# IST-DASLab/gptq-gguf-toolkit

Hardware: AMD Instinct MI355X
Metric: Mparams/s GPTQ-quantized (higher is better)
Workload: dtype f32; 1 GPU; llama3-8b-block-q4k: 7 Linears of one block (218.1 M params), 128x2048-token calibration fed per sequence through the package's BlockSchedule, block_size 128, rel_damp 0.01, nstep 20; calib_seqs_per_rank=128, parallelism=calib-dp1+matrix-fanout, owners=rank0

## Files before the change

gptq-gguf-toolkit_amd/csrc/gq_gptq.hip:

```cpp
#include <atomic>
#include <mutex>
#include "gq_common.hpp"
#include "gq_gemm32.hpp"
#include "gq_walk.hpp"
#include <stdlib.h>

namespace gq {

constexpr int SEG = 128;
constexpr int SB = 16;
constexpr int SEG_WAVES = 8;
constexpr int SEG_LDS_BYTES = (SEG * 64 + SEG * SEG + 2 * SB * 64) * 4 + SEG * 8;

__device__ __forceinline__ float div_rcp64(float n, double rd) { return (float)((double)n * rd); }

struct BandTable {
    int32_t n;
    int32_t end64[GQ_BANDS_MAX];
    uint32_t info[GQ_BANDS_MAX];
    int64_t sm_off[GQ_BANDS_MAX];
};
template <bool BANDS> struct BandArg {};
template <> struct BandArg<true> { BandTable t; };

template <bool PERM, bool UNI = false, bool BANDS = false>
__global__ __launch_bounds__(SEG_WAVES * 64) void gptq_segment_kernel(
    float* W, int64_t C, const float* src, int64_t ld_src,
    const float* __restrict__ U, int64_t a, int len, int64_t R,
    const uint16_t* __restrict__ d, const uint8_t* __restrict__ s, const uint16_t* __restrict__ dmin,
    const uint8_t* __restrict__ m, int G, int is_signed, float qmin, float qmax,
    uint8_t* __restrict__ qweight, float* __restrict__ Err, int64_t ld_err, int64_t err_col0,
    const int32_t* __restrict__ perm, const float* __restrict__ uscale = nullptr,
    const float* __restrict__ uzero = nullptr,
    const float* __restrict__ Unext = nullptr,
    int npair = 1,
    BandArg<BANDS> bands = {}) {
    extern __shared__ __attribute__((aligned(16))) float seg_smem[];
    float* wl = seg_smem;
    float* Us = seg_smem + SEG * 64;
    float* ne = Us + SEG * SEG;
    double* rdiag = reinterpret_cast<double*>(ne + 2 * SB * 64);
    const int tid = threadIdx.x, lane = tid & 63, wid = tid >> 6;
    const int64_t row = (int64_t)blockIdx.x * 64 + lane;
    const bool live = row < R;
    const int64_t r = live ? row : 0;
    int64_t band_row0 = 0;
    if constexpr (BANDS) {
        static_assert(!PERM && !UNI, "bands are K-quants in natural column order");
        const BandTable& bt = bands.t;
        int k = 0;
        while (k + 1 < bt.n && (int)blockIdx.x >= bt.end64[k]) ++k;
        const uint32_t info = bt.info[k];
        G = (int)(info & 0xffu);
        is_signed = (int)((info >> 8) & 1u);
        qmin = (float)(int8_t)((info >> 16) & 0xffu);
        qmax = (float)(info >> 24);
        band_row0 = k ? (int64_t)bt.end64[k - 1] * 64 : 0;
        s += bt.sm_off[k];
        m += bt.sm_off[k];
    }
    for (int half = 0; half < npair; ++half) {
    if (half) {
        __syncthreads();
        a += SEG;
        src += SEG;
        err_col0 += SEG;
        Unext = nullptr;
    }
    auto load_u_rows = [&](int i_lo, int i_hi, int t0, int nthr) {
        for (int idx = t0; idx < (i_hi - i_lo) * (SEG / 4); idx += nthr) {
            const int i = i_lo + idx / (SEG / 4), j4 = (idx % (SEG / 4)) * 4;
            float4 v = make_float4(0.f, 0.f, 0.f, 0.f);
            if (j4 < len) v = *reinterpret_cast<const float4*>(U + (a + i) * C + a + j4);
            *reinterpret_cast<float4*>(Us + i * SEG + j4) = v;
        }
    };
    auto load_w_cols = [&](int j_lo, int j_hi, int w0, int nw) {
        const float* sp = src + r * ld_src;
        for (int j = j_lo + w0 * 4; j < j_hi; j += 4 * nw) {
            float4 v = *reinterpret_cast<const float4*>(sp + j);
            wl[(j + 0) * 64 + lane] = v.x;
            wl[(j + 1) * 64 + lane] = v.y;
            wl[(j + 2) * 64 + lane] = v.z;
            wl[(j + 3) * 64 + lane] = v.w;
        }
    };
    const int first = len < SB ? len : SB;
    if (tid < first) rdiag[tid] = 1.0 / (double)U[(a + tid) * C + a + tid];
    load_u_rows(0, first, tid, SEG_WAVES * 64);
    load_w_cols(0, first, wid, SEG_WAVES);
    const int64_t nsg = C / 256, ng = C / G;
    constexpr int NT = SEG / SB;
    float dst[PERM ? 1 : NT], dmt[PERM ? 1 : NT];
    double rdt[PERM ? 1 : NT];
    if constexpr (!PERM) {
        if (wid == 0) {
#pragma unroll
            for (int t = 0; t < NT; ++t) {
                const int64_t col0 = a + t * SB < a + len ? a + t * SB : a;
                if constexpr (UNI) {
                    dst[t] = uscale[r * ng + col0 / G];
                    dmt[t] = uzero[r * ng + col0 / G];
                } else if constexpr (BANDS) {
                    const int64_t rb = r - band_row0;
                    dst[t] = h2f(d[r * nsg + col0 / 256]) * ival(s[rb * ng + col0 / G], is_signed);
                    dmt[t] = h2f(dmin[r * nsg + col0 / 256]) * ival(m[rb * ng + col0 / G], is_signed);
                } else {
                    dst[t] = h2f(d[r * nsg + col0 / 256]) * ival(s[r * ng + col0 / G], is_signed);
                    dmt[t] = h2f(dmin[r * nsg + col0 / 256]) * ival(m[r * ng + col0 / G], is_signed);
                }
                rdt[t] = 1.0 / (double)(dst[t] < 1e-9f ? 1e-9f : dst[t]);
            }
        }
    }
    __syncthreads();
    if (wid != 0) {
        const int ht = tid - 64;
        if (ht >= first && ht < len) rdiag[ht] = 1.0 / (double)U[(a + ht) * C + a + ht];
        load_u_rows(first, len, ht, (SEG_WAVES - 1) * 64);
        load_w_cols(first, len, wid - 1, SEG_WAVES - 1);
    }

    const int ntile = len / SB;
#pragma unroll
    for (int t = 0; t < NT; ++t) {
        if (t >= ntile) break;
        const int i0 = t * SB;
        float* net = ne + (t & 1) * (SB * 64);
        if (wid == 0) {
            const int64_t col0 = a + i0;
            float ds = 0.f, dm = 0.f, dsv[PERM ? SB : 1], dmv[PERM ? SB : 1];
            double rden = 0.0, rdenv[PERM ? SB : 1];
            if constexpr (PERM) {
#pragma unroll
                for (int k = 0; k < SB; ++k) {
                    const int64_t pc = perm[col0 + k];
                    dsv[k] = h2f(d[r * nsg + pc / 256]) * ival(s[r * ng + pc / G], is_signed);
                    dmv[k] = h2f(dmin[r * nsg + pc / 256]) * ival(m[r * ng + pc / G], is_signed);
                    rdenv[k] = 1.0 / (double)(dsv[k] < 1e-9f ? 1e-9f : dsv[k]);
                }
            } else {
                ds = dst[t];
                dm = dmt[t];
                rden = rdt[t];
            }
            float wr[SB], nerr[SB], wq[SB];
            uint32_t qpack[4] = {0, 0, 0, 0};
#pragma unroll
            for (int k = 0; k < SB; ++k) wr[k] = wl[(i0 + k) * 64 + lane];
#pragma unroll
            for (int k = 0; k < SB; ++k) {
                const float* urow = Us + (i0 + k) * SEG + i0;
                if constexpr (PERM) { ds = dsv[k]; dm = dmv[k]; rden = rdenv[k]; }
                float q;
                if constexpr (UNI) {
                    q = clampf(rintf(div_rcp64(wr[k], rden) + dm), qmin, qmax);
                    wq[k] = ds * (q - dm);
                } else {
                    q = clampf(rintf(div_rcp64(wr[k] + dm, rden)), qmin, qmax);
                    wq[k] = dequantize1(q, ds, dm);
                }
                const float err = div_rcp64(wr[k] - wq[k], rdiag[i0 + k]);
                const uint8_t qb = is_signed ? (uint8_t)(int8_t)q : (uint8_t)q;
                qpack[k >> 2] |= (uint32_t)qb << (8 * (k & 3));
                const float nk = -err;
                nerr[k] = nk;
#pragma unroll
                for (int kk = k; kk < SB; ++kk) wr[kk] = wr[kk] + nk * urow[kk];
            }
#pragma unroll
            for (int k = 0; k < SB; ++k) net[k * 64 + lane] = nerr[k];
            if (live) {
                *reinterpret_cast<uint4*>(qweight + row * C + col0) =
                    make_uint4(qpack[0], qpack[1], qpack[2], qpack[3]);
                float* wp = W + row * C + col0;
                float* ep = Err + row * ld_err + err_col0 + i0;
#pragma unroll
                for (int k = 0; k < SB; k += 4) {
                    *reinterpret_cast<float4*>(wp + k) = make_float4(wq[k], wq[k + 1], wq[k + 2], wq[k + 3]);
                    *reinterpret_cast<float4*>(ep + k) =
                        make_float4(-nerr[k], -nerr[k + 1], -nerr[k + 2], -nerr[k + 3]);
                }
            }
        }
        if (wid != 0 && t > 0) {
            const float* nep = ne + ((t - 1) & 1) * (SB * 64);
            if (Unext != nullptr && wid == SEG_WAVES - 1) {
#pragma unroll
                for (int k = 0; k < SB; ++k) wl[(i0 - SB + k) * 64 + lane] = nep[k * 64 + lane];
            }
            int turn = 0;
            for (int j0 = i0 + SB; j0 < len; j0 += SB, ++turn) {
                if ((turn % (SEG_WAVES - 1)) + 1 != wid) continue;
                float wt[SB], nk[SB];
#pragma unroll
                for (int jj = 0; jj < SB; ++jj) wt[jj] = wl[(j0 + jj) * 64 + lane];
#pragma unroll
                for (int k = 0; k < SB; ++k) nk[k] = nep[k * 64 + lane];
#pragma unroll
                for (int k = 0; k < SB; ++k) {
                    const float* urow = Us + (i0 - SB + k) * SEG + j0;
#pragma unroll
                    for (int jj = 0; jj < SB; ++jj) wt[jj] = wt[jj] + nk[k] * urow[jj];
                }
#pragma unroll
                for (int jj = 0; jj < SB; ++jj) wl[(j0 + jj) * 64 + lane] = wt[jj];
            }
        }
        __syncthreads();
        if (i0 + SB < len) {
            constexpr int CPW = SB / SEG_WAVES;
            const int j0 = i0 + SB + wid * CPW;
            float wt[CPW];
#pragma unroll
            for (int jj = 0; jj < CPW; ++jj) wt[jj] = wl[(j0 + jj) * 64 + lane];
#pragma unroll
            for (int k = 0; k < SB; ++k) {
                const float nk = net[k * 64 + lane];
#pragma unroll
                for (int jj = 0; jj < CPW; ++jj) wt[jj] = wt[jj] + nk * Us[(i0 + k) * SEG + j0 + jj];
            }
#pragma unroll
            for (int jj = 0; jj < CPW; ++jj) wl[(j0 + jj) * 64 + lane] = wt[jj];
        }
        __syncthreads();
    }
    if (Unext != nullptr) {
        for (int idx = tid; idx < SEG * (SEG / 4); idx += SEG_WAVES * 64) {
            const int i = idx / (SEG / 4), j4 = (idx % (SEG / 4)) * 4;
            *reinterpret_cast<float4*>(Us + i * SEG + j4) = *reinterpret_cast<const float4*>(Unext + (int64_t)i * C + j4);
        }
        __syncthreads();
        const int rb = (wid & 1) * 32, cb = (wid >> 1) * 32;
        const int li = lane & 31, lk = lane >> 5;
        const float* nel = ne + ((ntile - 1) & 1) * (SB * 64);
        f32x16 acc;
#pragma unroll
        for (int e = 0; e < 16; ++e) acc[e] = 0.0f;
#pragma unroll 8
        for (int k0 = 0; k0 < SEG; k0 += 2) {
            const int k = k0 + lk;
            const float ev = (k < SEG - SB) ? wl[k * 64 + rb + li] : nel[(k - (SEG - SB)) * 64 + rb + li];
            acc = __builtin_amdgcn_mfma_f32_32x32x2f32(ev, Us[k * SEG + cb + li], acc, 0, 0, 0);
        }
        const int64_t r0 = (int64_t)blockIdx.x * 64 + rb + 4 * lk;
        float* wp = W + r0 * C + a + SEG + cb + li;
        float wv[16];
#pragma unroll
        for (int e = 0; e < 16; ++e) {
            const int ro = (e & 3) + 8 * (e >> 2);
            wv[e] = (r0 + ro < R) ? wp[(int64_t)ro * C] : 0.0f;
        }
#pragma unroll
        for (int e = 0; e < 16; ++e) {
            const int ro = (e & 3) + 8 * (e >> 2);
            if (r0 + ro < R) wp[(int64_t)ro * C] = wv[e] + acc[e];
        }
    }
    }
}

__global__ __launch_bounds__(256) void uniform_params_kernel(const float* __restrict__ x, int64_t R, int64_t ld, int G,
                                                             float maxq, int sym, float* __restrict__ scale,
                                                             float* __restrict__ zero, int64_t ng) {
    const int lane = threadIdx.x & 63;
    const int64_t row = (int64_t)blockIdx.x * 4 + (threadIdx.x >> 6);
    if (row >= R) return;
    const float* xr = x + row * ld;
    float mn = xr[0], mx = mn;
    for (int j = lane * 4; j < G; j += 256) {
        const float4 v = *reinterpret_cast<const float4*>(xr + j);
        mn = fminf(fminf(mn, v.x), fminf(v.y, fminf(v.z, v.w)));
        mx = fmaxf(fmaxf(mx, v.x), fmaxf(v.y, fmaxf(v.z, v.w)));
    }
#pragma unroll
    for (int o = 32; o > 0; o >>= 1) {
        mn = fminf(mn, __shfl_xor(mn, o));
        mx = fmaxf(mx, __shfl_xor(mx, o));
    }
    if (lane) return;
    if (sym) {
        mx = fmaxf(fabsf(mn), mx);
        if (mn < 0.0f) mn = -mx;
    }
    if (mn == mx) {
        mn = -1.0f;
        mx = 1.0f;
    }
    const float sc = (mx - mn) / maxq;
    scale[row * ng] = sc;
    zero[row * ng] = sym ? (maxq + 1.0f) / 2.0f : rintf(-mn / sc);
}

__global__ __launch_bounds__(256) void block_far_update_kernel(float* __restrict__ Wblk, int64_t ld_blk,
                                                               int64_t ncols, int64_t R,
                                                               const float* __restrict__ Err, int64_t ld_err,
                                                               int64_t e0, int n_i, const float* __restrict__ U,
                                                               int64_t C, int64_t a, int64_t cj0) {
    const int64_t total = R * ncols;
    for (int64_t t = (int64_t)blockIdx.x * blockDim.x + threadIdx.x; t < total;
         t += (int64_t)gridDim.x * blockDim.x) {
        const int64_t r = t / ncols, j = t % ncols;
        float w = Wblk[r * ld_blk + j];
        const float* e = Err + r * ld_err + e0;
        for (int i = 0; i < n_i; ++i) w = w + (-e[i]) * U[(a + i) * C + cj0 + j];
        Wblk[r * ld_blk + j] = w;
    }
}

__global__ __launch_bounds__(256) void copy2d_kernel(float* __restrict__ dst, int64_t ld_dst,
                                                     const float* __restrict__ src, int64_t ld_src, int64_t R,
                                                     int64_t ncols) {
    const int64_t total = R * ncols;
    for (int64_t t = (int64_t)blockIdx.x * blockDim.x + threadIdx.x; t < total;
         t += (int64_t)gridDim.x * blockDim.x) {
        const int64_t r = t / ncols, j = t % ncols;
        dst[r * ld_dst + j] = src[r * ld_src + j];
    }
}

int launch_trailing_update(float* Cmat, int64_t ldc, const float* A, int64_t lda, const float* B, int64_t ldb,
                           int64_t M, int64_t N, int64_t K, hipStream_t st) {
    ProfScope ps(PT_TRAILING, st);
    return launch_gemm32<false, 0, false>(Cmat, ldc, A, lda, B, ldb, M, N, K, st);
}

constexpr int LA = 8;
constexpr int LA_B = 128;

static std::atomic<int> g_far_enabled{1};
int far_helper_enable(int on) { return g_far_enabled.exchange(on ? 1 : 0); }

WalkOptions walk_options() {
    return WalkOptions{opt(OPT_la), opt(OPT_no_lookahead), opt(OPT_far_sync), opt(OPT_far_async_max_rows),
                       opt(OPT_far_async_min_sb), opt(OPT_far_wgs), opt(OPT_near64_maxn), g_far_enabled.load() != 0};
}

WalkPlan walk_plan(int64_t R, int64_t C, int block_size, WalkKind kind, int uniform_group, const WalkOptions& o) {
    WalkPlan p{};
    const int64_t B = p.B = block_size <= 0 || block_size > C ? C : block_size;
    p.la = (o.la >= 2 && o.la <= LA && o.la % 2 == 0) ? (int)o.la : LA;
    const int ug = kind == WalkKind::Uniform && uniform_group > 0 ? uniform_group : 0;
    p.lookahead = B == LA_B && !o.no_lookahead && (!ug || (p.la * B) % ug == 0);
    p.pair_look = p.lookahead && p.la % 2 == 0 && (!ug || 256 % ug == 0);
    p.ldE = p.lookahead ? (int64_t)LA * B : B;
    p.helper_ok = p.lookahead && o.helper_enabled && !o.far_sync && R % 128 == 0 && C % 128 == 0 &&
                  R <= o.far_async_max_rows && C >= o.far_async_min_sb * (int64_t)p.la * B;
    p.far_wgs = (int)o.far_wgs;
    p.near64_maxn = o.near64_maxn;
    const size_t blk = (size_t)R * (size_t)B * sizeof(float);
    const size_t err = blk * (B == LA_B ? 2 * (size_t)LA : 1);
    p.needs_blk = B > SEG || (B > 0 && 256 % B != 0);
    p.err_off[0] = 0;
    p.err_off[1] = B == LA_B ? blk * LA : 0;
    p.blk_off = err;
    p.panel_off = (err + (p.needs_blk ? blk : 0) + 255) & ~(size_t)255;
    p.total = err + (p.needs_blk ? blk : 0) + 256 + 256;
    return p;
}

size_t gptq_workspace_bytes(int64_t R, int64_t C, int block_size) {
    return walk_plan(R, C, block_size, WalkKind::KQuant, 0, walk_options()).total;
}
int gptq_uses_helper_stream(int64_t R, int64_t C, int block_size) {
    return walk_plan(R, C, block_size, WalkKind::KQuant, 0, walk_options()).helper_ok;
}

struct BandPlan {
    BandTable tbl;
    int q_type[GQ_BANDS_MAX];
    int64_t row_end[GQ_BANDS_MAX];
};

enum class ScaleSearch {
    None,
    UpFront,
    Lazy,
};

struct Walk {
    const WalkCall& c;
    WalkPlan p;
    TypeInfo ti;
    ScaleSearch search;
    float *err[2], *Wblk;
    unsigned* panel;
    int64_t ng, nsg;
    int gps;
    bool helper;
};
struct Block {
    int64_t c1, c2;
    int64_t sb, pos;
    int64_t S0, S1;
    bool single;
    float* Err;
};

static int walk_open(const WalkCall& c, Walk& w) {
    const bool uni = c.kind == WalkKind::Uniform;
    w.ti = TypeInfo{};
    if (uni) {
        w.ti.group = c.uni.group > 0 ? c.uni.group : (int)c.C;
        w.ti.qmax = (1 << c.uni.bits) - 1;
    } else if (c.kind == WalkKind::Bands) {
        w.ti.group = 16;
        for (int k = 0; k < c.bands->tbl.n; ++k) {
            TypeInfo tk;
            type_info(c.bands->q_type[k], tk);
            w.ti.k_search |= tk.k_search;
        }
    } else if (!type_info(c.q_type, w.ti)) GQ_FAIL(GQ_E_BAD_TYPE, "gq_gptq_quantize: unknown q_type %d", c.q_type);
    if (c.R <= 0 || c.C <= 0 || c.C % 256)
// ... 389 lines not shown
```

Baseline: 2432 Mparams/s.

## Hand over paired segment in LDS instead of reloading, add stamp profiling

Moves the segment kernel into its own header and changes the paired-block path (non-uniform quants). After the first 128-column block, the trailing update results for the partner block are written straight into the LDS working buffer, and the next U tile and its diagonal reciprocals are prefetched. The second half therefore skips its prologue reload and the extra barrier. The commit also adds an optional s_memtime stamp template parameter and a micro-profiler program. This removes global-memory round trips and a sync at the hand-over, at the cost of more complex LDS bookkeeping and higher register pressure.

```diff
diff --git a/gptq-gguf-toolkit_amd/csrc/gq_gptq.hip b/gptq-gguf-toolkit_amd/csrc/gq_gptq.hip
--- a/gptq-gguf-toolkit_amd/csrc/gq_gptq.hip
+++ b/gptq-gguf-toolkit_amd/csrc/gq_gptq.hip
@@ -3,262 +3,10 @@
 #include "gq_common.hpp"
 #include "gq_gemm32.hpp"
 #include "gq_walk.hpp"
+#include "gq_segment.hpp"
 #include <stdlib.h>
 
 namespace gq {
-
-constexpr int SEG = 128;
-constexpr int SB = 16;
-constexpr int SEG_WAVES = 8;
-constexpr int SEG_LDS_BYTES = (SEG * 64 + SEG * SEG + 2 * SB * 64) * 4 + SEG * 8;
-
-__device__ __forceinline__ float div_rcp64(float n, double rd) { return (float)((double)n * rd); }
-
-struct BandTable {
-    int32_t n;
-    int32_t end64[GQ_BANDS_MAX];
-    uint32_t info[GQ_BANDS_MAX];
-    int64_t sm_off[GQ_BANDS_MAX];
-};
-template <bool BANDS> struct BandArg {};
-template <> struct BandArg<true> { BandTable t; };
-
-template <bool PERM, bool UNI = false, bool BANDS = false>
-__global__ __launch_bounds__(SEG_WAVES * 64) void gptq_segment_kernel(
-    float* W, int64_t C, const float* src, int64_t ld_src,
-    const float* __restrict__ U, int64_t a, int len, int64_t R,
-    const uint16_t* __restrict__ d, const uint8_t* __restrict__ s, const uint16_t* __restrict__ dmin,
-    const uint8_t* __restrict__ m, int G, int is_signed, float qmin, float qmax,
-    uint8_t* __restrict__ qweight, float* __restrict__ Err, int64_t ld_err, int64_t err_col0,
-    const int32_t* __restrict__ perm, const float* __restrict__ uscale = nullptr,
-    const float* __restrict__ uzero = nullptr,
-    const float* __restrict__ Unext = nullptr,
-    int npair = 1,
-    BandArg<BANDS> bands = {}) {
-    extern __shared__ __attribute__((aligned(16))) float seg_smem[];
-    float* wl = seg_smem;
-    float* Us = seg_smem + SEG * 64;
-    float* ne = Us + SEG * SEG;
-    double* rdiag = reinterpret_cast<double*>(ne + 2 * SB * 64);
-    const int tid = threadIdx.x, lane = tid & 63, wid = tid >> 6;
-    const int64_t row = (int64_t)blockIdx.x * 64 + lane;
-    const bool live = row < R;
-    const int64_t r = live ? row : 0;
-    int64_t band_row0 = 0;
-    if constexpr (BANDS) {
-        static_assert(!PERM && !UNI, "bands are K-quants in natural column order");
-        const BandTable& bt = bands.t;
-        int k = 0;
-        while (k + 1 < bt.n && (int)blockIdx.x >= bt.end64[k]) ++k;
-        const uint32_t info = bt.info[k];
-        G = (int)(info & 0xffu);
-        is_signed = (int)((info >> 8) & 1u);
-        qmin = (float)(int8_t)((info >> 16) & 0xffu);
-        qmax = (float)(info >> 24);
-        band_row0 = k ? (int64_t)bt.end64[k - 1] * 64 : 0;
-        s += bt.sm_off[k];
-        m += bt.sm_off[k];
-    }
-    for (int half = 0; half < npair; ++half) {
-    if (half) {
-        __syncthreads();
-        a += SEG;
-        src += SEG;
-        err_col0 += SEG;
-        Unext = nullptr;
-    }
-    auto load_u_rows = [&](int i_lo, int i_hi, int t0, int nthr) {
-        for (int idx = t0; idx < (i_hi - i_lo) * (SEG / 4); idx += nthr) {
-            const int i = i_lo + idx / (SEG / 4), j4 = (idx % (SEG / 4)) * 4;
-            float4 v = make_float4(0.f, 0.f, 0.f, 0.f);
-            if (j4 < len) v = *reinterpret_cast<const float4*>(U + (a + i) * C + a + j4);
-            *reinterpret_cast<float4*>(Us + i * SEG + j4) = v;
-        }
-    };
-    auto load_w_cols = [&](int j_lo, int j_hi, int w0, int nw) {
-        const float* sp = src + r * ld_src;
-        for (int j = j_lo + w0 * 4; j < j_hi; j += 4 * nw) {
-            float4 v = *reinterpret_cast<const float4*>(sp + j);
-            wl[(j + 0) * 64 + lane] = v.x;
-            wl[(j + 1) * 64 + lane] = v.y;
-            wl[(j + 2) * 64 + lane] = v.z;
-            wl[(j + 3) * 64 + lane] = v.w;
-        }
-    };
-    const int first = len < SB ? len : SB;
-    if (tid < first) rdiag[tid] = 1.0 / (double)U[(a + tid) * C + a + tid];
-    load_u_rows(0, first, tid, SEG_WAVES * 64);
-    load_w_cols(0, first, wid, SEG_WAVES);
-    const int64_t nsg = C / 256, ng = C / G;
-    constexpr int NT = SEG / SB;
-    float dst[PERM ? 1 : NT], dmt[PERM ? 1 : NT];
-    double rdt[PERM ? 1 : NT];
-    if constexpr (!PERM) {
-        if (wid == 0) {
-#pragma unroll
-            for (int t = 0; t < NT; ++t) {
-                const int64_t col0 = a + t * SB < a + len ? a + t * SB : a;
-                if constexpr (UNI) {
-                    dst[t] = uscale[r * ng + col0 / G];
-                    dmt[t] = uzero[r * ng + col0 / G];
-                } else if constexpr (BANDS) {
-                    const int64_t rb = r - band_row0;
-                    dst[t] = h2f(d[r * nsg + col0 / 256]) * ival(s[rb * ng + col0 / G], is_signed);
-                    dmt[t] = h2f(dmin[r * nsg + col0 / 256]) * ival(m[rb * ng + col0 / G], is_signed);
-                } else {
-                    dst[t] = h2f(d[r * nsg + col0 / 256]) * ival(s[r * ng + col0 / G], is_signed);
-                    dmt[t] = h2f(dmin[r * nsg + col0 / 256]) * ival(m[r * ng + col0 / G], is_signed);
-                }
-                rdt[t] = 1.0 / (double)(dst[t] < 1e-9f ? 1e-9f : dst[t]);
-            }
-        }
-    }
-    __syncthreads();
-    if (wid != 0) {
-        const int ht = tid - 64;
-        if (ht >= first && ht < len) rdiag[ht] = 1.0 / (double)U[(a + ht) * C + a + ht];
-        load_u_rows(first, len, ht, (SEG_WAVES - 1) * 64);
-        load_w_cols(first, len, wid - 1, SEG_WAVES - 1);
-    }
-
-    const int ntile = len / SB;
-#pragma unroll
-    for (int t = 0; t < NT; ++t) {
-        if (t >= ntile) break;
-        const int i0 = t * SB;
-        float* net = ne + (t & 1) * (SB * 64);
-        if (wid == 0) {
-            const int64_t col0 = a + i0;
-            float ds = 0.f, dm = 0.f, dsv[PERM ? SB : 1], dmv[PERM ? SB : 1];
-            double rden = 0.0, rdenv[PERM ? SB : 1];
-            if constexpr (PERM) {
-#pragma unroll
-                for (int k = 0; k < SB; ++k) {
-                    const int64_t pc = perm[col0 + k];
-                    dsv[k] = h2f(d[r * nsg + pc / 256]) * ival(s[r * ng + pc / G], is_signed);
-                    dmv[k] = h2f(dmin[r * nsg + pc / 256]) * ival(m[r * ng + pc / G], is_signed);
-                    rdenv[k] = 1.0 / (double)(dsv[k] < 1e-9f ? 1e-9f : dsv[k]);
-                }
-            } else {
-                ds = dst[t];
-                dm = dmt[t];
-                rden = rdt[t];
-            }
-            float wr[SB], nerr[SB], wq[SB];
-            uint32_t qpack[4] = {0, 0, 0, 0};
-#pragma unroll
-            for (int k = 0; k < SB; ++k) wr[k] = wl[(i0 + k) * 64 + lane];
-#pragma unroll
-            for (int k = 0; k < SB; ++k) {
-                const float* urow = Us + (i0 + k) * SEG + i0;
-                if constexpr (PERM) { ds = dsv[k]; dm = dmv[k]; rden = rdenv[k]; }
-                float q;
-                if constexpr (UNI) {
-                    q = clampf(rintf(div_rcp64(wr[k], rden) + dm), qmin, qmax);
-                    wq[k] = ds * (q - dm);
-                } else {
-                    q = clampf(rintf(div_rcp64(wr[k] + dm, rden)), qmin, qmax);
-                    wq[k] = dequantize1(q, ds, dm);
-                }
-                const float err = div_rcp64(wr[k] - wq[k], rdiag[i0 + k]);
-                const uint8_t qb = is_signed ? (uint8_t)(int8_t)q : (uint8_t)q;
-                qpack[k >> 2] |= (uint32_t)qb << (8 * (k & 3));
-                const float nk = -err;
-                nerr[k] = nk;
-#pragma unroll
-                for (int kk = k; kk < SB; ++kk) wr[kk] = wr[kk] + nk * urow[kk];
-            }
-#pragma unroll
-            for (int k = 0; k < SB; ++k) net[k * 64 + lane] = nerr[k];
-            if (live) {
-                *reinterpret_cast<uint4*>(qweight + row * C + col0) =
-                    make_uint4(qpack[0], qpack[1], qpack[2], qpack[3]);
-                float* wp = W + row * C + col0;
-                float* ep = Err + row * ld_err + err_col0 + i0;
-#pragma unroll
-                for (int k = 0; k < SB; k += 4) {
-                    *reinterpret_cast<float4*>(wp + k) = make_float4(wq[k], wq[k + 1], wq[k + 2], wq[k + 3]);
-                    *reinterpret_cast<float4*>(ep + k) =
-                        make_float4(-nerr[k], -nerr[k + 1], -nerr[k + 2], -nerr[k + 3]);
-                }
-            }
-        }
-        if (wid != 0 && t > 0) {
-            const float* nep = ne + ((t - 1) & 1) * (SB * 64);
-            if (Unext != nullptr && wid == SEG_WAVES - 1) {
-#pragma unroll
-                for (int k = 0; k < SB; ++k) wl[(i0 - SB + k) * 64 + lane] = nep[k * 64 + lane];
-            }
-            int turn = 0;
-            for (int j0 = i0 + SB; j0 < len; j0 += SB, ++turn) {
-                if ((turn % (SEG_WAVES - 1)) + 1 != wid) continue;
-                float wt[SB], nk[SB];
-#pragma unroll
-                for (int jj = 0; jj < SB; ++jj) wt[jj] = wl[(j0 + jj) * 64 + lane];
-#pragma unroll
-                for (int k = 0; k < SB; ++k) nk[k] = nep[k * 64 + lane];
-#pragma unroll
-                for (int k = 0; k < SB; ++k) {
-                    const float* urow = Us + (i0 - SB + k) * SEG + j0;
-#pragma unroll
-                    for (int jj = 0; jj < SB; ++jj) wt[jj] = wt[jj] + nk[k] * urow[jj];
-                }
-#pragma unroll
-                for (int jj = 0; jj < SB; ++jj) wl[(j0 + jj) * 64 + lane] = wt[jj];
-            }
-        }
-        __syncthreads();
-        if (i0 + SB < len) {
-            constexpr int CPW = SB / SEG_WAVES;
-            const int j0 = i0 + SB + wid * CPW;
-            float wt[CPW];
-#pragma unroll
-            for (int jj = 0; jj < CPW; ++jj) wt[jj] = wl[(j0 + jj) * 64 + lane];
-#pragma unroll
-            for (int k = 0; k < SB; ++k) {
-                const float nk = net[k * 64 + lane];
-#pragma unroll
-                for (int jj = 0; jj < CPW; ++jj) wt[jj] = wt[jj] + nk * Us[(i0 + k) * SEG + j0 + jj];
-            }
-#pragma unroll
-            for (int jj = 0; jj < CPW; ++jj) wl[(j0 + jj) * 64 + lane] = wt[jj];
-        }
-        __syncthreads();
-    }
-    if (Unext != nullptr) {
-        for (int idx = tid; idx < SEG * (SEG / 4); idx += SEG_WAVES * 64) {
-            const int i = idx / (SEG / 4), j4 = (idx % (SEG / 4)) * 4;
-            *reinterpret_cast<float4*>(Us + i * SEG + j4) = *reinterpret_cast<const float4*>(Unext + (int64_t)i * C + j4);
-        }
-        __syncthreads();
-        const int rb = (wid & 1) * 32, cb = (wid >> 1) * 32;
-        const int li = lane & 31, lk = lane >> 5;
-        const float* nel = ne + ((ntile - 1) & 1) * (SB * 64);
-        f32x16 acc;
-#pragma unroll
-        for (int e = 0; e < 16; ++e) acc[e] = 0.0f;
-#pragma unroll 8
-        for (int k0 = 0; k0 < SEG; k0 += 2) {
-            const int k = k0 + lk;
-            const float ev = (k < SEG - SB) ? wl[k * 64 + rb + li] : nel[(k - (SEG - SB)) * 64 + rb + li];
-            acc = __builtin_amdgcn_mfma_f32_32x32x2f32(ev, Us[k * SEG + cb + li], acc, 0, 0, 0);
-        }
-        const int64_t r0 = (int64_t)blockIdx.x * 64 + rb + 4 * lk;
-        float* wp = W + r0 * C + a + SEG + cb + li;
-        float wv[16];
-#pragma unroll
-        for (int e = 0; e < 16; ++e) {
-            const int ro = (e & 3) + 8 * (e >> 2);
-            wv[e] = (r0 + ro < R) ? wp[(int64_t)ro * C] : 0.0f;
-        }
-#pragma unroll
-        for (int e = 0; e < 16; ++e) {
-            const int ro = (e & 3) + 8 * (e >> 2);
-            if (r0 + ro < R) wp[(int64_t)ro * C] = wv[e] + acc[e];
-        }
-    }
-    }
-}
 
 __global__ __launch_bounds__(256) void uniform_params_kernel(const float* __restrict__ x, int64_t R, int64_t ld, int G,
                                                              float maxq, int sym, float* __restrict__ scale,
diff --git a/gptq-gguf-toolkit_amd/csrc/gq_segment.hpp b/gptq-gguf-toolkit_amd/csrc/gq_segment.hpp
--- /dev/null
+++ b/gptq-gguf-toolkit_amd/csrc/gq_segment.hpp
@@ -0,0 +1,352 @@
+#pragma once
+#include "gq_common.hpp"
+#include "gq_gemm32.hpp"
+#include "../../include/gptq_gguf_levels.h"
+
+namespace gq {
+
+constexpr int SEG = 128;
+constexpr int SB = 16;
+constexpr int SEG_WAVES = 8;
+constexpr int SEG_LDS_BYTES = (SEG * 64 + SEG * SEG + 2 * SB * 64) * 4 + SEG * 8;
+
+__device__ __forceinline__ float div_rcp64(float n, double rd) { return (float)((double)n * rd); }
+
+struct BandTable {
+    int32_t n;
+    int32_t end64[GQ_BANDS_MAX];
+    uint32_t info[GQ_BANDS_MAX];
+    int64_t sm_off[GQ_BANDS_MAX];
+};
+template <bool BANDS> struct BandArg {};
+template <> struct BandArg<true> { BandTable t; };
+
+constexpr int SEG_STAMP_HALF = 24, SEG_NSTAMP = 2 * SEG_STAMP_HALF + 4;
+template <bool STAMP> struct StampArg {};
+template <> struct StampArg<true> { unsigned long long* buf; int wg; };
+
+template <bool PERM, bool UNI = false, bool BANDS = false, bool STAMP = false>
+__global__ __launch_bounds__(SEG_WAVES * 64) void gptq_segment_kernel(
+    float* W, int64_t C, const float* src, int64_t ld_src,
+    const float* __restrict__ U, int64_t a, int len, int64_t R,
+    const uint16_t* __restrict__ d, const uint8_t* __restrict__ s, const uint16_t* __restrict__ dmin,
+    const uint8_t* __restrict__ m, int G, int is_signed, float qmin, float qmax,
+    uint8_t* __restrict__ qweight, float* __restrict__ Err, int64_t ld_err, int64_t err_col0,
+    const int32_t* __restrict__ perm, const float* __restrict__ uscale = nullptr,
+    const float* __restrict__ uzero = nullptr,
+    const float* __restrict__ Unext = nullptr,
+    int npair = 1,
+    BandArg<BANDS> bands = {}, StampArg<STAMP> stamp = {}) {
+    extern __shared__ __attribute__((aligned(16))) float seg_smem[];
+    float* wl = seg_smem;
+    float* Us = seg_smem + SEG * 64;
+    float* ne = Us + SEG * SEG;
+    double* rdiag = reinterpret_cast<double*>(ne + 2 * SB * 64);
+    const int tid = threadIdx.x, lane = tid & 63, wid = tid >> 6;
+    const int64_t row = (int64_t)blockIdx.x * 64 + lane;
+    const bool live = row < R;
+    const int64_t r = live ? row : 0;
+    int stamp_base = 0;
+    auto stamp_at = [&](int point) {
+        if constexpr (STAMP) {
+            if ((int)blockIdx.x == stamp.wg) {
+                unsigned long long t_;
+                asm volatile("s_memtime %0\n\ts_waitcnt lgkmcnt(0)" : "=s"(t_)::"memory");
+                if (lane == 0) stamp.buf[wid * SEG_NSTAMP + stamp_base + point] = t_;
+            }
+        }
+    };
+    auto stamp_wall = [&](int slot) {
+        if constexpr (STAMP) {
+            if ((int)blockIdx.x == stamp.wg && tid == 0) stamp.buf[SEG_NSTAMP - 2 + slot] = __builtin_amdgcn_s_memrealtime();
+        }
+    };
+    stamp_wall(0);
+    int64_t band_row0 = 0;
+    if constexpr (BANDS) {
+        static_assert(!PERM && !UNI, "bands are K-quants in natural column order");
+        const BandTable& bt = bands.t;
+        int k = 0;
+        while (k + 1 < bt.n && (int)blockIdx.x >= bt.end64[k]) ++k;
+        const uint32_t info = bt.info[k];
+        G = (int)(info & 0xffu);
+        is_signed = (int)((info >> 8) & 1u);
+        qmin = (float)(int8_t)((info >> 16) & 0xffu);
+        qmax = (float)(info >> 24);
+        band_row0 = k ? (int64_t)bt.end64[k - 1] * 64 : 0;
+        s += bt.sm_off[k];
+        m += bt.sm_off[k];
+    }
+    constexpr int NT = SEG / SB;
+    float dst[PERM ? 1 : NT], dmt[PERM ? 1 : NT];
+    double rdt[PERM ? 1 : NT];
+    for (int half = 0; half < npair; ++half) {
+    if (half) {
+        if constexpr (UNI) __syncthreads();
+        a += SEG;
+        src += SEG;
+        err_col0 += SEG;
+        Unext = nullptr;
+        stamp_base = SEG_STAMP_HALF;
+    }
+    const bool pair = !UNI && Unext != nullptr, handed = !UNI && half == 1;
+    stamp_at(0);
+    auto load_u_rows = [&](int i_lo, int i_hi, int t0, int nthr) {
+        for (int idx = t0; idx < (i_hi - i_lo) * (SEG / 4); idx += nthr) {
+            const int i = i_lo + idx / (SEG / 4), j4 = (idx % (SEG / 4)) * 4;
+            float4 v = make_float4(0.f, 0.f, 0.f, 0.f);
+            if (j4 < len) v = *reinterpret_cast<const float4*>(U + (a + i) * C + a + j4);
+            *reinterpret_cast<float4*>(Us + i * SEG + j4) = v;
+        }
+    };
+    auto load_w_cols = [&](int j_lo, int j_hi, int w0, int nw) {
+        const float* sp = src + r * ld_src;
+        for (int j = j_lo + w0 * 4; j < j_hi; j += 4 * nw) {
+            float4 v = *reinterpret_cast<const float4*>(sp + j);
+            wl[(j + 0) * 64 + lane] = v.x;
+            wl[(j + 1) * 64 + lane] = v.y;
+            wl[(j + 2) * 64 + lane] = v.z;
+            wl[(j + 3) * 64 + lane] = v.w;
+        }
+    };
+    const int first = len < SB ? len : SB;
+    if (!handed) {
+        if (tid < first) rdiag[tid] = 1.0 / (double)U[(a + tid) * C + a + tid];
+        load_u_rows(0, first, tid, SEG_WAVES * 64);
+        load_w_cols(0, first, wid, SEG_WAVES);
+    }
+    const int64_t nsg = C / 256, ng = C / G;
+    auto group_params = [&](int64_t a0) {
+        if constexpr (!PERM) {
+#pragma unroll
+            for (int t = 0; t < NT; ++t) {
+                const int64_t col0 = a0 + t * SB < a0 + len ? a0 + t * SB : a0;
+                if constexpr (UNI) {
+                    dst[t] = uscale[r * ng + col0 / G];
+                    dmt[t] = uzero[r * ng + col0 / G];
+                } else if constexpr (BANDS) {
+                    const int64_t rb = r - band_row0;
+                    dst[t] = h2f(d[r * nsg + col0 / 256]) * ival(s[rb * ng + col0 / G], is_signed);
+                    dmt[t] = h2f(dmin[r * nsg + col0 / 256]) * ival(m[rb * ng + col0 / G], is_signed);
+                } else {
+                    dst[t] = h2f(d[r * nsg + col0 / 256]) * ival(s[r * ng + col0 / G], is_signed);
+                    dmt[t] = h2f(dmin[r * nsg + col0 / 256]) * ival(m[r * ng + col0 / G], is_signed);
+                }
+                rdt[t] = 1.0 / (double)(dst[t] < 1e-9f ? 1e-9f : dst[t]);
+            }
+        }
+    };
+    if (wid == 0 && !handed) group_params(a);
+    __syncthreads();
+    stamp_at(1);
+    if (wid != 0) {
+        const int ht = tid - 64;
+        if (ht >= first && ht < len) rdiag[ht] = 1.0 / (double)U[(a + ht) * C + a + ht];
+        load_u_rows(first, len, ht, (SEG_WAVES - 1) * 64);
+        if (!handed) load_w_cols(first, len, wid - 1, SEG_WAVES - 1);
+    }
+
+    const int ntile = len / SB;
+#pragma unroll
+    for (int t = 0; t < NT; ++t) {
+        if (t >= ntile) break;
+        const int i0 = t * SB;
+        float* net = ne + (t & 1) * (SB * 64);
+        if (wid == 0) {
+            const int64_t col0 = a + i0;
+            float ds = 0.f, dm = 0.f, dsv[PERM ? SB : 1], dmv[PERM ? SB : 1];
+            double rden = 0.0, rdenv[PERM ? SB : 1];
+            if constexpr (PERM) {
+#pragma unroll
+                for (int k = 0; k < SB; ++k) {
+                    const int64_t pc = perm[col0 + k];
+                    dsv[k] = h2f(d[r * nsg + pc / 256]) * ival(s[r * ng + pc / G], is_signed);
+                    dmv[k] = h2f(dmin[r * nsg + pc / 256]) * ival(m[r * ng + pc / G], is_signed);
+                    rdenv[k] = 1.0 / (double)(dsv[k] < 1e-9f ? 1e-9f : dsv[k]);
+                }
+            } else {
+                ds = dst[t];
+                dm = dmt[t];
+                rden = rdt[t];
+            }
+            float wr[SB], nerr[SB], wq[SB];
+            uint32_t qpack[4] = {0, 0, 0, 0};
+#pragma unroll
+            for (int k = 0; k < SB; ++k) wr[k] = wl[(i0 + k) * 64 + lane];
+#pragma unroll
+            for (int k = 0; k < SB; ++k) {
+                const float* urow = Us + (i0 + k) * SEG + i0;
+                if constexpr (PERM) { ds = dsv[k]; dm = dmv[k]; rden = rdenv[k]; }
+                float q;
+                if constexpr (UNI) {
+                    q = clampf(rintf(div_rcp64(wr[k], rden) + dm), qmin, qmax);
+                    wq[k] = ds * (q - dm);
+                } else {
+                    q = clampf(rintf(div_rcp64(wr[k] + dm, rden)), qmin, qmax);
+                    wq[k] = dequantize1(q, ds, dm);
+                }
+                const float err = div_rcp64(wr[k] - wq[k], rdiag[i0 + k]);
+                const uint8_t qb = is_signed ? (uint8_t)(int8_t)q : (uint8_t)q;
+                qpack[k >> 2] |= (uint32_t)qb << (8 * (k & 3));
+                const float nk = -err;
+                nerr[k] = nk;
+#pragma unroll
+                for (int kk = k; kk < SB; ++kk) wr[kk] = wr[kk] + nk * urow[kk];
+            }
+#pragma unroll
+            for (int k = 0; k < SB; ++k) net[k * 64 + lane] = nerr[k];
+            if (live) {
+                *reinterpret_cast<uint4*>(qweight + row * C + col0) =
+                    make_uint4(qpack[0], qpack[1], qpack[2], qpack[3]);
+                float* wp = W + row * C + col0;
+                float* ep = Err + row * ld_err + err_col0 + i0;
+#pragma unroll
+                for (int k = 0; k < SB; k += 4) {
+                    *reinterpret_cast<float4*>(wp + k) = make_float4(wq[k], wq[k + 1], wq[k + 2], wq[k + 3]);
+                    *reinterpret_cast<float4*>(ep + k) =
+                        make_float4(-nerr[k], -nerr[k + 1], -nerr[k + 2], -nerr[k + 3]);
+                }
+            }
+        }
+        if constexpr (!UNI) {
+            if (pair && t == NT - 1 && wid != 0) {
+                for (int idx = tid - 64; idx < (SEG - SB) * (SEG / 4); idx += (SEG_WAVES - 1) * 64) {
+                    const int i = idx / (SEG / 4), j4 = (idx % (SEG / 4)) * 4;
+                    *reinterpret_cast<float4*>(Us + i * SEG + j4) = *reinterpret_cast<const float4*>(Unext + (int64_t)i * C + j4);
+                }
+            }
+        }
+        if (wid != 0 && t > 0) {
+            const float* nep = ne + ((t - 1) & 1) * (SB * 64);
+            if (Unext != nullptr && wid == SEG_WAVES - 1) {
+#pragma unroll
+                for (int k = 0; k < SB; ++k) wl[(i0 - SB + k) * 64 + lane] = nep[k * 64 + lane];
+            }
+            int turn = 0;
+            for (int j0 = i0 + SB; j0 < len; j0 += SB, ++turn) {
+                if ((turn % (SEG_WAVES - 1)) + 1 != wid) continue;
+                float wt[SB], nk[SB];
+#pragma unroll
+                for (int jj = 0; jj < SB; ++jj) wt[jj] = wl[(j0 + jj) * 64 + lane];
+#pragma unroll
+                for (int k = 0; k < SB; ++k) nk[k] = nep[k * 64 + lane];
+#pragma unroll
+                for (int k = 0; k < SB; ++k) {
+                    const float* urow = Us + (i0 - SB + k) * SEG + j0;
+#pragma unroll
+                    for (int jj = 0; jj < SB; ++jj) wt[jj] = wt[jj] + nk[k] * urow[jj];
+                }
+#pragma unroll
+                for (int jj = 0; jj < SB; ++jj) wl[(j0 + jj) * 64 + lane] = wt[jj];
+            }
+        }
+        stamp_at(2 + 2 * t);
+        __syncthreads();
+        if (i0 + SB < len) {
+            constexpr int CPW = SB / SEG_WAVES;
+            const int j0 = i0 + SB + wid * CPW;
+            float wt[CPW];
+#pragma unroll
+            for (int jj = 0; jj < CPW; ++jj) wt[jj] = wl[(j0 + jj) * 64 + lane];
+#pragma unroll
+            for (int k = 0; k < SB; ++k) {
+                const float nk = net[k * 64 + lane];
+#pragma unroll
+                for (int jj = 0; jj < CPW; ++jj) wt[jj] = wt[jj] + nk * Us[(i0 + k) * SEG + j0 + jj];
+            }
+#pragma unroll
+            for (int jj = 0; jj < CPW; ++jj) wl[(j0 + jj) * 64 + lane] = wt[jj];
+        }
+        if (!(pair && t == NT - 1)) __syncthreads();
+        stamp_at(3 + 2 * t);
+    }
+    if constexpr (!UNI) {
+        if (pair) {
+            stamp_at(18);
+            const int rb = (wid & 1) * 32, cb = (wid >> 1) * 32;
+            const int li = lane & 31, lk = lane >> 5;
+            const int ui = tid / (SEG / 4), uj4 = (tid % (SEG / 4)) * 4;
+            const float4 ul = *reinterpret_cast<const float4*>(Unext + (int64_t)(SEG - SB + ui) * C + uj4);
+            const int64_t r0 = (int64_t)blockIdx.x * 64 + rb + 4 * lk;
+            const float* wp = W + r0 * C + a + SEG + cb + li;
+            float wv[16];
+#pragma unroll
+            for (int e = 0; e < 16; ++e) {
+                const int ro = (e & 3) + 8 * (e >> 2);
+                wv[e] = (r0 + ro < R) ? wp[(int64_t)ro * C] : 0.0f;
+            }
+            const float4 un = *reinterpret_cast<const float4*>(U + (a + SEG + ui) * C + a + SEG + uj4);
+            float dg = 1.0f;
+            if (tid < SB) dg = U[(a + SEG + tid) * C + a + SEG + tid];
+            if (wid == 0) group_params(a + SEG);
+            f32x16 acc;
+#pragma unroll
+            for (int e = 0; e < 16; ++e) acc[e] = 0.0f;
+#pragma unroll 8
+            for (int k0 = 0; k0 < SEG - SB; k0 += 2) {
+                const int k = k0 + lk;
+                acc = __builtin_amdgcn_mfma_f32_32x32x2f32(wl[k * 64 + rb + li], Us[k * SEG + cb + li], acc, 0, 0, 0);
+            }
+            *reinterpret_cast<float4*>(Us + (SEG - SB + ui) * SEG + uj4) = ul;
+            __syncthreads();
+            const float* nel = ne + ((NT - 1) & 1) * (SB * 64);
+#pragma unroll
+            for (int k0 = SEG - SB; k0 < SEG; k0 += 2) {
+                const int k = k0 + lk;
+                acc = __builtin_amdgcn_mfma_f32_32x32x2f32(nel[(k - (SEG - SB)) * 64 + rb + li], Us[k * SEG + cb + li], acc, 0, 0, 0);
+            }
+            stamp_at(19);
+            float* wc = wl + (cb + li) * 64 + rb + 4 * lk;
+#pragma unroll
+            for (int q = 0; q < 4; ++q) {
+                float v[4];
+#pragma unroll
+                for (int i = 0; i < 4; ++i) v[i] = (r0 + 8 * q + i < R) ? wv[4 * q + i] + acc[4 * q + i] : 0.0f;
+                *reinterpret_cast<float4*>(wc + 8 * q) = make_float4(v[0], v[1], v[2], v[3]);
+            }
+            *reinterpret_cast<float4*>(Us + ui * SEG + uj4) = un;
+            if (tid < SB) rdiag[tid] = 1.0 / (double)dg;
+            stamp_at(20);
+        }
+    } else if (Unext != nullptr) {
+        for (int idx = tid; idx < SEG * (SEG / 4); idx += SEG_WAVES * 64) {
+            const int i = idx / (SEG / 4), j4 = (idx % (SEG / 4)) * 4;
+            *reinterpret_cast<float4*>(Us + i * SEG + j4) = *reinterpret_cast<const float4*>(Unext + (int64_t)i * C + j4);
+        }
+        __syncthreads();
+        stamp_at(18);
+        const int rb = (wid & 1) * 32, cb = (wid >> 1) * 32;
+        const int li = lane & 31, lk = lane >> 5;
+        const float* nel = ne + ((ntile - 1) & 1) * (SB * 64);
+        f32x16 acc;
+#pragma unroll
+        for (int e = 0; e < 16; ++e) acc[e] = 0.0f;
+#pragma unroll 8
+        for (int k0 = 0; k0 < SEG; k0 += 2) {
+            const int k = k0 + lk;
+            const float ev = (k < SEG - SB) ? wl[k * 64 + rb + li] : nel[(k - (SEG - SB)) * 64 + rb + li];
+            acc = __builtin_amdgcn_mfma_f32_32x32x2f32(ev, Us[k * SEG + cb + li], acc, 0, 0, 0);
+        }
+        stamp_at(19);
+        const int64_t r0 = (int64_t)blockIdx.x * 64 + rb + 4 * lk;
+        float* wp = W + r0 * C + a + SEG + cb + li;
+        float wv[16];
+#pragma unroll
+        for (int e = 0; e < 16; ++e) {
+            const int ro = (e & 3) + 8 * (e >> 2);
+            wv[e] = (r0 + ro < R) ? wp[(int64_t)ro * C] : 0.0f;
+        }
+#pragma unroll
+        for (int e = 0; e < 16; ++e) {
+            const int ro = (e & 3) + 8 * (e >> 2);
+            if (r0 + ro < R) wp[(int64_t)ro * C] = wv[e] + acc[e];
+        }
+        stamp_at(20);
+    }
+    }
+    stamp_base = 0;
+    stamp_at(2 * SEG_STAMP_HALF);
+    stamp_wall(1);
+}
+
+}
diff --git a/profiles/micro/pair_stamps.hip b/profiles/micro/pair_stamps.hip
--- /dev/null
+++ b/profiles/micro/pair_stamps.hip
@@ -0,0 +1,120 @@
+#include "../../gptq-gguf-toolkit_amd/csrc/gq_segment.hpp"
+#include <algorithm>
+#include <vector>
+namespace gq {
+thread_local char g_err[512];
+unsigned g_prof_mask = 0;
+void prof_begin(int, hipStream_t) {}
+void prof_end(int, hipStream_t) {}
+int64_t opt(Opt) { return 0; }
+}
+using namespace gq;
+#define CK(x) do { hipError_t e_ = (x); if (e_ != hipSuccess) { printf("%s: %s\n", #x, hipGetErrorString(e_)); return 1; } } while (0)
+
+struct Problem {
+    float *W, *U, *Err;
+    uint16_t *d, *dmin;
+    uint8_t *s, *m, *q;
+    int64_t R, C, a;
+};
+
+template <bool STAMP>
+static void launch(const Problem& p, unsigned long long* st, int wg) {
+    StampArg<STAMP> sa;
+    if constexpr (STAMP) { sa.buf = st; sa.wg = wg; }
+    hipLaunchKernelGGL((gptq_segment_kernel<false, false, false, STAMP>), dim3((unsigned)(p.R / 64)), dim3(SEG_WAVES * 64),
+                       SEG_LDS_BYTES, 0, p.W, p.C, p.W + p.a, p.C, p.U, p.a, SEG, p.R, p.d, p.s, p.dmin, p.m, 32, 0, 0.0f, 15.0f,
+                       p.q, p.Err, (int64_t)1024, (int64_t)0, nullptr, nullptr, nullptr, p.U + p.a * p.C + p.a + SEG, 2,
+                       BandArg<false>{}, sa);
+}
+
+template <bool STAMP>
+static float best_us(const Problem& p, unsigned long long* st, int wg, int reps) {
+    hipEvent_t e0, e1; hipEventCreate(&e0); hipEventCreate(&e1);
+    float best = 1e9f;
+    for (int r = 0; r < 30; ++r) launch<STAMP>(p, st, wg);
+    for (int r = 0; r < reps; ++r) {
+        hipEventRecord(e0);
+        launch<STAMP>(p, st, wg);
+        hipEventRecord(e1); hipEventSynchronize(e1);
+        float ms; hipEventElapsedTime(&ms, e0, e1);
+        best = std::min(best, ms);
+    }
+    return best * 1e3f;
+}
+
+int main() {
+    Problem p;
+    p.R = 4096; p.C = 14336; p.a = 7168;
+    const int64_t R = p.R, C = p.C, nsg = C / 256, ng = C / 32;
+    unsigned long long* st;
+    CK(hipMalloc(&p.W, R * C * 4)); CK(hipMalloc(&p.U, C * C * 4)); CK(hipMalloc(&p.Err, R * 1024 * 4));
+    CK(hipMalloc(&p.d, R * nsg * 2)); CK(hipMalloc(&p.dmin, R * nsg * 2)); CK(hipMalloc(&p.s, R * ng)); CK(hipMalloc(&p.m, R * ng));
+    CK(hipMalloc(&p.q, R * C)); CK(hipMalloc(&st, SEG_WAVES * SEG_NSTAMP * 8));
+    CK(hipMemset(p.U, 0, C * C * 4));
+    srand(1);
+    {
+        std::vector<float> u((size_t)256 * C, 0.0f);
+        for (int i = 0; i < 256; ++i)
+            for (int64_t j = p.a + i; j < p.a + 256; ++j) u[(size_t)i * C + j] = j == p.a + i ? 1.0f : 0.01f * (rand() / (float)RAND_MAX - 0.5f);
+        CK(hipMemcpy(p.U + p.a * C, u.data(), u.size() * 4, hipMemcpyHostToDevice));
+        std::vector<float> w((size_t)R * C);
+        for (auto& x : w) x = 0.04f * (rand() / (float)RAND_MAX - 0.5f);
+        CK(hipMemcpy(p.W, w.data(), w.size() * 4, hipMemcpyHostToDevice));
+        std::vector<uint16_t> d((size_t)R * nsg, 0x10c5), dm((size_t)R * nsg, 0x0cc5);
+        std::vector<uint8_t> sm((size_t)R * ng);
+        for (auto& x : sm) x = (uint8_t)(1 + rand() % 63);
+        CK(hipMemcpy(p.d, d.data(), d.size() * 2, hipMemcpyHostToDevice)); CK(hipMemcpy(p.dmin, dm.data(), dm.size() * 2, hipMemcpyHostToDevice));
+        CK(hipMemcpy(p.s, sm.data(), sm.size(), hipMemcpyHostToDevice)); CK(hipMemcpy(p.m, sm.data(), sm.size(), hipMemcpyHostToDevice));
+    }
+    CK(hipFuncSetAttribute((const void*)gptq_segment_kernel<false, false, false, false>, hipFuncAttributeMaxDynamicSharedMemorySize, SEG_LDS_BYTES));
+    CK(hipFuncSetAttribute((const void*)gptq_segment_kernel<false, false, false, true>, hipFuncAttributeMaxDynamicSharedMemorySize, SEG_LDS_BYTES));
+    const int wg = (int)(R / 128);
+    const float plain = best_us<false>(p, st, wg, 20);
+    CK(hipMemset(st, 0, SEG_WAVES * SEG_NSTAMP * 8));
+    const float stamped = best_us<true>(p, st, wg, 20);
+    CK(hipDeviceSynchronize());
+    std::vector<unsigned long long> h(SEG_WAVES * SEG_NSTAMP);
+    CK(hipMemcpy(h.data(), st, h.size() * 8, hipMemcpyDeviceToHost));
+    const int H = SEG_STAMP_HALF, END = 2 * H;
+    const unsigned long long t0 = h[0];
+    const double cyc = (double)(h[END] - t0), wall_us = (double)(h[SEG_NSTAMP - 1] - h[SEG_NSTAMP - 2]) / 100.0;
+    const double us = wall_us / cyc;
+    auto w0 = [&](int pt) { return (double)(h[pt] - t0) * us; };
+    auto helpers = [&](int pt) {
+        unsigned long long mx = 0;
+        for (int w = 1; w < SEG_WAVES; ++w) mx = std::max(mx, h[w * SEG_NSTAMP + pt]);
+        return (double)(mx - t0) * us;
+    };
+    printf("pair launch 4096 x 14336 Q4_K, columns %ld .. %ld: plain %.1f us, with stamps %.1f us\n", (long)p.a, (long)p.a + 255, plain, stamped);
+    printf("stamped workgroup %d: %.1f us from its first to its last stamp, shader clock %.3f GHz\n", wg, wall_us, 1e-3 / us);
+    printf("%-44s %9s %9s %9s\n", "phase (wave 0)", "us", "ends at", "helpers");
+    double chain = 0.0, bound = 0.0;
+    auto row = [&](const char* name, int from, int to) {
+        printf("%-44s %9.2f %9.2f %9.2f\n", name, w0(to) - w0(from), w0(to), helpers(to));
+    };
+    char nm[64];
+    for (int half = 0; half < 2; ++half) {
+        const int b = half * H;
+        if (half == 0) row("prologue 0", 0, 1);
+        else row("second prologue (up to first partner column)", 20, b + 1);
+        for (int t = 0; t < 8; ++t) {
+            snprintf(nm, sizeof nm, "block %d tile %d chain", half, t);
+            row(nm, b + 1 + 2 * t, b + 2 + 2 * t);
+            snprintf(nm, sizeof nm, "block %d tile %d boundary", half, t);
+            row(nm, b + 2 + 2 * t, b + 3 + 2 * t);
+            chain += w0(b + 2 + 2 * t) - w0(b + 1 + 2 * t);
+            bound += w0(b + 3 + 2 * t) - w0(b + 2 + 2 * t);
+        }
+        if (half == 0) {
+            row("last even column -> Unext in LDS", 16, 18);
+            row("MFMAs", 18, 19);
+            row("partner's working values updated", 19, 20);
+        }
+    }
+    row("tail", H + 17, END);
+    printf("sums: chains %.2f us, tile boundaries %.2f us (the last boundary of block 0 is part of the hand-over)\n", chain, bound);
+    printf("hand-over: last even column -> first partner column %.2f us = %.1f %% of the workgroup's %.1f us\n", w0(H + 1) - w0(16),
+           100.0 * (w0(H + 1) - w0(16)) / wall_us, wall_us);
+    return 0;
+}
```

Result: no change. 2432 Mparams/s (-0.0%).

## Stage per-tile quant scales in LDS and cut register pressure in GPTQ segment kernel

Applied to the files above, without the earlier changes.

Per-tile scale/min/reciprocal values move from per-thread register arrays into new LDS slots, and per-row pointers for d/dmin/s/m and uniform params are hoisted out of the pair loop. The tile loop is no longer unrolled, and asm barriers keep tid, len and C in chosen register classes, all aimed at lowering VGPR pressure and spills. The PERM path loads perm indices once per lane and broadcasts them with shuffles, and an explicit waitcnt is placed before the W read-modify-write. The cost is a small increase in LDS use, extra LDS reads per tile, and a loop that may schedule less well than the fully unrolled one.

```diff
diff --git a/gptq-gguf-toolkit_amd/csrc/gq_gptq.hip b/gptq-gguf-toolkit_amd/csrc/gq_gptq.hip
--- a/gptq-gguf-toolkit_amd/csrc/gq_gptq.hip
+++ b/gptq-gguf-toolkit_amd/csrc/gq_gptq.hip
@@ -10,7 +10,8 @@
 constexpr int SEG = 128;
 constexpr int SB = 16;
 constexpr int SEG_WAVES = 8;
-constexpr int SEG_LDS_BYTES = (SEG * 64 + SEG * SEG + 2 * SB * 64) * 4 + SEG * 8;
+constexpr int SEG_NT = SEG / SB;
+constexpr int SEG_LDS_BYTES = (SEG * 64 + SEG * SEG + 2 * SB * 64) * 4 + SEG * 8 + SEG_NT * 64 * 16;
 
 __device__ __forceinline__ float div_rcp64(float n, double rd) { return (float)((double)n * rd); }
 
@@ -40,10 +41,9 @@
     float* Us = seg_smem + SEG * 64;
     float* ne = Us + SEG * SEG;
     double* rdiag = reinterpret_cast<double*>(ne + 2 * SB * 64);
-    const int tid = threadIdx.x, lane = tid & 63, wid = tid >> 6;
-    const int64_t row = (int64_t)blockIdx.x * 64 + lane;
-    const bool live = row < R;
-    const int64_t r = live ? row : 0;
+    double* rdg = rdiag + SEG;
+    float* dsg = reinterpret_cast<float*>(rdg + SEG_NT * 64);
+    float* dmg = dsg + SEG_NT * 64;
     int64_t band_row0 = 0;
     if constexpr (BANDS) {
         static_assert(!PERM && !UNI, "bands are K-quants in natural column order");
@@ -59,6 +59,14 @@
         s += bt.sm_off[k];
         m += bt.sm_off[k];
     }
+    const int64_t nsg = C / 256, ng = C / G;
+    const int64_t prow = (int64_t)blockIdx.x * 64 + (threadIdx.x & 63), pr = prow < R ? prow : 0;
+    const uint16_t* const drow = UNI ? nullptr : d + pr * nsg;
+    const uint16_t* const dminrow = UNI ? nullptr : dmin + pr * nsg;
+    const uint8_t* const srow = UNI ? nullptr : s + (pr - band_row0) * ng;
+    const uint8_t* const mrow = UNI ? nullptr : m + (pr - band_row0) * ng;
+    const float* const uscrow = UNI ? uscale + pr * ng : nullptr;
+    const float* const uzrow = UNI ? uzero + pr * ng : nullptr;
     for (int half = 0; half < npair; ++half) {
     if (half) {
         __syncthreads();
@@ -67,11 +75,19 @@
         err_col0 += SEG;
         Unext = nullptr;
     }
+    int tid = threadIdx.x;
+    asm volatile("" : "+v"(tid));
+    int lenq = len;
+    asm volatile("" : "+s"(lenq));
+    const int lane = tid & 63, wid = tid >> 6;
+    const int64_t row = (int64_t)blockIdx.x * 64 + lane;
+    const bool live = row < R;
+    const int64_t r = live ? row : 0;
     auto load_u_rows = [&](int i_lo, int i_hi, int t0, int nthr) {
         for (int idx = t0; idx < (i_hi - i_lo) * (SEG / 4); idx += nthr) {
             const int i = i_lo + idx / (SEG / 4), j4 = (idx % (SEG / 4)) * 4;
             float4 v = make_float4(0.f, 0.f, 0.f, 0.f);
-            if (j4 < len) v = *reinterpret_cast<const float4*>(U + (a + i) * C + a + j4);
+            if (j4 < lenq) v = *reinterpret_cast<const float4*>(U + (a + i) * C + a + j4);
             *reinterpret_cast<float4*>(Us + i * SEG + j4) = v;
         }
     };
@@ -85,46 +101,51 @@
             wl[(j + 3) * 64 + lane] = v.w;
         }
     };
-    const int first = len < SB ? len : SB;
+    const int first = lenq < SB ? lenq : SB;
     if (tid < first) rdiag[tid] = 1.0 / (double)U[(a + tid) * C + a + tid];
     load_u_rows(0, first, tid, SEG_WAVES * 64);
     load_w_cols(0, first, wid, SEG_WAVES);
-    const int64_t nsg = C / 256, ng = C / G;
-    constexpr int NT = SEG / SB;
-    float dst[PERM ? 1 : NT], dmt[PERM ? 1 : NT];
-    double rdt[PERM ? 1 : NT];
+    constexpr int NT = SEG_NT;
     if constexpr (!PERM) {
         if (wid == 0) {
+            const int64_t ga = a / G;
+            const int ra = (int)(a - ga * G);
+            float st[NT], mt[NT], dsup = 0.f, dminsup = 0.f;
+            if constexpr (!UNI) {
+                dsup = h2f(drow[a / 256]);
+                dminsup = h2f(dminrow[a / 256]);
+            }
 #pragma unroll
             for (int t = 0; t < NT; ++t) {
-                const int64_t col0 = a + t * SB < a + len ? a + t * SB : a;
+                const int64_t gi = ga + (ra + (t * SB < lenq ? t * SB : 0)) / G;
                 if constexpr (UNI) {
-                    dst[t] = uscale[r * ng + col0 / G];
-                    dmt[t] = uzero[r * ng + col0 / G];
-                } else if constexpr (BANDS) {
-                    const int64_t rb = r - band_row0;
-                    dst[t] = h2f(d[r * nsg + col0 / 256]) * ival(s[rb * ng + col0 / G], is_signed);
-                    dmt[t] = h2f(dmin[r * nsg + col0 / 256]) * ival(m[rb * ng + col0 / G], is_signed);
+                    st[t] = uscrow[gi];
+                    mt[t] = uzrow[gi];
                 } else {
-                    dst[t] = h2f(d[r * nsg + col0 / 256]) * ival(s[r * ng + col0 / G], is_signed);
-                    dmt[t] = h2f(dmin[r * nsg + col0 / 256]) * ival(m[r * ng + col0 / G], is_signed);
+                    st[t] = ival(srow[gi], is_signed);
+                    mt[t] = ival(mrow[gi], is_signed);
                 }
-                rdt[t] = 1.0 / (double)(dst[t] < 1e-9f ? 1e-9f : dst[t]);
+            }
+#pragma unroll
+            for (int t = 0; t < NT; ++t) {
+                const float dst = UNI ? st[t] : dsup * st[t], dmt = UNI ? mt[t] : dminsup * mt[t];
+                dsg[t * 64 + lane] = dst;
+                dmg[t * 64 + lane] = dmt;
+                rdg[t * 64 + lane] = 1.0 / (double)(dst < 1e-9f ? 1e-9f : dst);
             }
         }
     }
     __syncthreads();
     if (wid != 0) {
         const int ht = tid - 64;
-        if (ht >= first && ht < len) rdiag[ht] = 1.0 / (double)U[(a + ht) * C + a + ht];
-        load_u_rows(first, len, ht, (SEG_WAVES - 1) * 64);
-        load_w_cols(first, len, wid - 1, SEG_WAVES - 1);
+        if (ht >= first && ht < lenq) rdiag[ht] = 1.0 / (double)U[(a + ht) * C + a + ht];
+        load_u_rows(first, lenq, ht, (SEG_WAVES - 1) * 64);
+        load_w_cols(first, lenq, wid - 1, SEG_WAVES - 1);
     }
 
     const int ntile = len / SB;
-#pragma unroll
-    for (int t = 0; t < NT; ++t) {
-        if (t >= ntile) break;
+#pragma unroll 1
+    for (int t = 0; t < ntile; ++t) {
         const int i0 = t * SB;
         float* net = ne + (t & 1) * (SB * 64);
         if (wid == 0) {
@@ -132,17 +153,18 @@
             float ds = 0.f, dm = 0.f, dsv[PERM ? SB : 1], dmv[PERM ? SB : 1];
             double rden = 0.0, rdenv[PERM ? SB : 1];
             if constexpr (PERM) {
+                const int pcl = perm[col0 + (lane & (SB - 1))], sgl = pcl / 256, gl = pcl / G;
 #pragma unroll
                 for (int k = 0; k < SB; ++k) {
-                    const int64_t pc = perm[col0 + k];
-                    dsv[k] = h2f(d[r * nsg + pc / 256]) * ival(s[r * ng + pc / G], is_signed);
-                    dmv[k] = h2f(dmin[r * nsg + pc / 256]) * ival(m[r * ng + pc / G], is_signed);
+                    const int sg = __shfl(sgl, k), g = __shfl(gl, k);
+                    dsv[k] = h2f(drow[sg]) * ival(srow[g], is_signed);
+                    dmv[k] = h2f(dminrow[sg]) * ival(mrow[g], is_signed);
                     rdenv[k] = 1.0 / (double)(dsv[k] < 1e-9f ? 1e-9f : dsv[k]);
                 }
             } else {
-                ds = dst[t];
-                dm = dmt[t];
-                rden = rdt[t];
+                ds = dsg[t * 64 + lane];
+                dm = dmg[t * 64 + lane];
+                rden = rdg[t * 64 + lane];
             }
             float wr[SB], nerr[SB], wq[SB];
             uint32_t qpack[4] = {0, 0, 0, 0};
@@ -244,17 +266,20 @@
             acc = __builtin_amdgcn_mfma_f32_32x32x2f32(ev, Us[k * SEG + cb + li], acc, 0, 0, 0);
         }
         const int64_t r0 = (int64_t)blockIdx.x * 64 + rb + 4 * lk;
-        float* wp = W + r0 * C + a + SEG + cb + li;
+        int64_t Cq = C;
+        asm volatile("" : "+s"(Cq));
+        float* wp = W + r0 * Cq + a + SEG + cb + li;
         float wv[16];
 #pragma unroll
         for (int e = 0; e < 16; ++e) {
             const int ro = (e & 3) + 8 * (e >> 2);
-            wv[e] = (r0 + ro < R) ? wp[(int64_t)ro * C] : 0.0f;
-        }
+            wv[e] = (r0 + ro < R) ? wp[(int64_t)ro * Cq] : 0.0f;
+        }
+        __builtin_amdgcn_s_waitcnt(0x0f70);
 #pragma unroll
         for (int e = 0; e < 16; ++e) {
             const int ro = (e & 3) + 8 * (e >> 2);
-            if (r0 + ro < R) wp[(int64_t)ro * C] = wv[e] + acc[e];
+            if (r0 + ro < R) wp[(int64_t)ro * Cq] = wv[e] + acc[e];
         }
     }
     }
```

Result: faster. 2470 Mparams/s before, 2498 Mparams/s after, median of 6 (+1.1%).
